# IuvenisSapiens/Qwen3-TTS-Rust

Hardware: AMD Instinct MI355X
Metric: audio-seconds generated per second (aggregate over GPUs) = concurrent real-time streams; RTF and first-chunk latency from the single-utterance leg (higher is better)
Workload: dtype i8

## Files before the change

### qwen3-tts-rust_amd/csrc/codec.hip

```cpp
#include "codec.h"
#include "gguf.h"
#include <cmath>
#include <cstdlib>
#include <map>

namespace q3 {

typedef float f32x16 __attribute__((ext_vector_type(16)));

enum { EPI_NONE = 0, EPI_GELU = 1, EPI_RES_SCALE = 2, EPI_RES = 3, EPI_SNAKE = 4 };

struct GemmArgs {
    const float* A; int lda;
    int cin, dil;
    const float* W;
    const float* bias;
    float* out; int ldo;
    int M, N, K;
    int epi; const float* res; int ldr; const float* scale;
    const float *snake_ea, *snake_ib;
    float* ws;
    int a_segT, a_skip; int o_segT; long long o_skip; int r_segT; long long r_skip;
    int a_split, o_split;
    int xcd_swizzle;
};
#define SEG_NONE 0x3fffffff

__device__ __forceinline__ int seg_of(int row, int segT) { return segT == SEG_NONE ? 0 : row / segT; }
__device__ __forceinline__ size_t out_off(const GemmArgs& g, int row, int col) { return (size_t)row * g.ldo + (size_t)seg_of(row, g.o_segT) * g.o_skip + col; }
typedef _Float16 h4v_ __attribute__((ext_vector_type(4)));
__device__ __forceinline__ float4 load_a4(const GemmArgs& g, size_t row, int ci) {
    if (!g.a_split) return *reinterpret_cast<const float4*>(g.A + row * g.lda + ci);
    const _Float16* base = reinterpret_cast<const _Float16*>(g.A + row * g.lda);
    const h4v_ hi = *reinterpret_cast<const h4v_*>(base + ci), lo = *reinterpret_cast<const h4v_*>(base + g.cin + ci);
    return make_float4((float)hi[0] + (float)lo[0], (float)hi[1] + (float)lo[1], (float)hi[2] + (float)lo[2], (float)hi[3] + (float)lo[3]);
}
__device__ __forceinline__ float4 load_a4_split_raw(const GemmArgs& g, size_t row, int ci) {
    const _Float16* base = reinterpret_cast<const _Float16*>(g.A + row * g.lda);
    const float2 hi = *reinterpret_cast<const float2*>(base + ci), lo = *reinterpret_cast<const float2*>(base + g.cin + ci);
    return make_float4(hi.x, hi.y, lo.x, lo.y);
}
__device__ __forceinline__ void gemm_store(const GemmArgs& g, int row, int col, float v) {
    const size_t o = out_off(g, row, 0);
    if (!g.o_split) { g.out[o + col] = v; return; }
    _Float16* base = reinterpret_cast<_Float16*>(g.out + o);
    const _Float16 hi = (_Float16)v;
    base[col] = hi; base[g.N + col] = (_Float16)(v - (float)hi);
}

__device__ __forceinline__ float snake_sin(float x) {
    const float n = rintf(x * 0.63661977236758134f);
    float r = fmaf(n, -1.57079637050628662f, x);
    r = fmaf(n, 4.37113900018624283e-8f, r);
    const int q = (int)n;
    const float r2 = r * r;
    const float sp = fmaf(fmaf(fmaf(-1.9515295891e-4f, r2, 8.3321608736e-3f), r2, -1.6666654611e-1f), r2 * r, r);
    const float cp = fmaf(fmaf(fmaf(2.443315711809948e-5f, r2, -1.388731625493765e-3f), r2, 4.166664568298827e-2f), r2 * r2, fmaf(-0.5f, r2, 1.0f));
    const float v = (q & 1) ? cp : sp;
    return (q & 2) ? -v : v;
}
__device__ __forceinline__ float gemm_epilogue(const GemmArgs& g, float v, int row, int col) {
    if (g.bias) v += g.bias[col];
    if (g.epi == EPI_GELU) v = 0.5f * v * (1.0f + erff(v * 0.70710678118654752f));
    else if (g.epi == EPI_RES_SCALE) v = g.res[(size_t)row * g.ldr + (size_t)seg_of(row, g.r_segT) * g.r_skip + col] + g.scale[col] * v;
    else if (g.epi == EPI_RES) v = g.res[(size_t)row * g.ldr + (size_t)seg_of(row, g.r_segT) * g.r_skip + col] + v;
    else if (g.epi == EPI_SNAKE) { const float sn = snake_sin(v * g.snake_ea[col]); v = v + g.snake_ib[col] * (sn * sn); }
    return v;
}

typedef _Float16 h4e_ __attribute__((ext_vector_type(4)));
__device__ __forceinline__ void gemm_epilogue_store4(const GemmArgs& g, float4 t, int row, int col) {
    float v[4] = {t.x, t.y, t.z, t.w};
    if (g.bias) { const float4 b = *reinterpret_cast<const float4*>(g.bias + col); v[0] += b.x; v[1] += b.y; v[2] += b.z; v[3] += b.w; }
    if (g.epi == EPI_GELU) {
#pragma unroll
        for (int c = 0; c < 4; c++) v[c] = 0.5f * v[c] * (1.0f + erff(v[c] * 0.70710678118654752f));
    } else if (g.epi == EPI_RES_SCALE || g.epi == EPI_RES) {
        const float4 rs = *reinterpret_cast<const float4*>(g.res + (size_t)row * g.ldr + (size_t)seg_of(row, g.r_segT) * g.r_skip + col);
        if (g.epi == EPI_RES_SCALE) {
            const float4 sc = *reinterpret_cast<const float4*>(g.scale + col);
            v[0] = rs.x + sc.x * v[0]; v[1] = rs.y + sc.y * v[1]; v[2] = rs.z + sc.z * v[2]; v[3] = rs.w + sc.w * v[3];
        } else { v[0] = rs.x + v[0]; v[1] = rs.y + v[1]; v[2] = rs.z + v[2]; v[3] = rs.w + v[3]; }
    } else if (g.epi == EPI_SNAKE) {
        const float4 ea = *reinterpret_cast<const float4*>(g.snake_ea + col), ib = *reinterpret_cast<const float4*>(g.snake_ib + col);
        const float eav[4] = {ea.x, ea.y, ea.z, ea.w}, ibv[4] = {ib.x, ib.y, ib.z, ib.w};
#pragma unroll
        for (int c = 0; c < 4; c++) { const float sn = snake_sin(v[c] * eav[c]); v[c] = v[c] + ibv[c] * (sn * sn); }
    }
    const size_t o = out_off(g, row, 0);
    if (!g.o_split) *reinterpret_cast<float4*>(g.out + o + col) = make_float4(v[0], v[1], v[2], v[3]);
    else {
        _Float16* base = reinterpret_cast<_Float16*>(g.out + o);
        h4e_ hi, lo;
#pragma unroll
        for (int c = 0; c < 4; c++) { hi[c] = (_Float16)v[c]; lo[c] = (_Float16)(v[c] - (float)hi[c]); }
        *reinterpret_cast<h4e_*>(base + col) = hi;
        *reinterpret_cast<h4e_*>(base + g.N + col) = lo;
    }
}
static bool epilogue4_ok(const GemmArgs& g) {
    auto a16 = [](const void* p) { return (reinterpret_cast<uintptr_t>(p) & 15) == 0; };
    return g.N % 4 == 0 && g.ldo % 4 == 0 && g.o_skip % 4 == 0 && a16(g.out) && (!g.bias || a16(g.bias)) &&
           (!(g.epi == EPI_RES || g.epi == EPI_RES_SCALE) || (g.ldr % 4 == 0 && g.r_skip % 4 == 0 && a16(g.res))) &&
           (g.epi != EPI_RES_SCALE || a16(g.scale)) && (g.epi != EPI_SNAKE || (a16(g.snake_ea) && a16(g.snake_ib)));
}

template <int WM>
__global__ void __launch_bounds__(256) k_conv_gemm(GemmArgs g) {
    constexpr int WN = 4 / WM, BM = 32 * WM, BN = 32 * WN, BK = 16;
    constexpr int NA = BM * 4 / 256 > 0 ? BM * 4 / 256 : 1, NB = BN * 4 / 256 > 0 ? BN * 4 / 256 : 1;
    __shared__ float As[BK][BM];
    __shared__ float Bs[BK][BN];
    const int tid = threadIdx.x, lane = tid & 63, wave = tid >> 6;
    const int wm = wave / WN, wn = wave % WN;
    const int m0 = blockIdx.y * BM, n0 = blockIdx.x * BN;
    const int ksplit = gridDim.z, kper = g.K / ksplit, kbeg = blockIdx.z * kper, kend = kbeg + kper;
    f32x16 acc;
#pragma unroll
    for (int i = 0; i < 16; i++) acc[i] = 0.0f;
    float4 ra[NA], rb[NB];
    int arow[NA];
#pragma unroll
    for (int i = 0; i < NA; i++) { const int mm = m0 + (tid + i * 256) % BM; arow[i] = mm + seg_of(mm, g.a_segT) * g.a_skip; }
    auto fetch = [&](int k0) {
        const int j = k0 / g.cin, ci0 = k0 % g.cin;
#pragma unroll
        for (int i = 0; i < NA; i++) {
            const int e = tid + i * 256, r = e % BM, qd = e / BM;
            ra[i] = make_float4(0.f, 0.f, 0.f, 0.f);
            if (e < BM * 4 && m0 + r < g.M) ra[i] = load_a4(g, (size_t)(arow[i] + j * g.dil), ci0 + 4 * qd);
        }
#pragma unroll
        for (int i = 0; i < NB; i++) {
            const int e = tid + i * 256, r = e % BN, qd = e / BN;
            rb[i] = make_float4(0.f, 0.f, 0.f, 0.f);
            if (e < BN * 4 && n0 + r < g.N) rb[i] = *reinterpret_cast<const float4*>(g.W + (size_t)(n0 + r) * g.K + k0 + 4 * qd);
        }
// ... 368 lines not shown
            const int kk = 4 * (lane + 64 * i);
            w4[i] = (kk < kt) ? *reinterpret_cast<const float4*>(g.W + (size_t)nn * g.K + k0 + kk) : make_float4(0.f, 0.f, 0.f, 0.f);
        }
        __syncthreads();
        for (int e = tid; e < MT * (KT / 4); e += 512) {
            const int m = e / (KT / 4), kk = 4 * (e % (KT / 4));
            float4 v = make_float4(0.f, 0.f, 0.f, 0.f);
            if (m < g.M && kk < kt) {
                const int kg = k0 + kk, j = kg / g.cin, ci = kg % g.cin;
                v = load_a4(g, (size_t)(m + seg_of(m, g.a_segT) * g.a_skip + j * g.dil), ci);
            }
            *reinterpret_cast<float4*>(&As[m][kk]) = v;
        }
        __syncthreads();
#pragma unroll
        for (int i = 0; i < 2; i++) {
            const int kk = 4 * (lane + 64 * i);
#pragma unroll
            for (int m = 0; m < MT; m++) {
                const float4 a = *reinterpret_cast<const float4*>(&As[m][kk]);
                acc[m] += w4[i].x * a.x + w4[i].y * a.y + w4[i].z * a.z + w4[i].w * a.w;
            }
        }
    }
    float mine = 0.0f;
#pragma unroll
    for (int m = 0; m < MT; m++) {
        float v = acc[m];
        for (int o = 32; o >= 1; o >>= 1) v += __shfl_xor(v, o);
        if (lane == m) mine = v;
    }
    if (lane < MT && lane < g.M && n < g.N) gemm_store(g, lane, n, gemm_epilogue(g, mine, lane, n));
}
static const bool g_codec_f32 = [] { const char* e = std::getenv("Q3_CODEC_F32"); return e && e[0] == '1'; }();
static void gemm(hipStream_t st, GemmArgs g, float* ws, size_t ws_floats, const _Float16* wh = nullptr, const _Float16* wl = nullptr) {
    if (g.M <= 16) {
        dim3 grid((g.N + 7) / 8);
        if (g.M <= 4) hipLaunchKernelGGL((k_skinny_gemm<4>), grid, dim3(512), 0, st, g);
        else if (g.M <= 8) hipLaunchKernelGGL((k_skinny_gemm<8>), grid, dim3(512), 0, st, g);
        else hipLaunchKernelGGL((k_skinny_gemm<16>), grid, dim3(512), 0, st, g);
        return;
    }
    const bool small = g.M <= 32;
    const int tiles = small ? ((g.N + 127) / 128) * ((g.M + 31) / 32) : ((g.N + 63) / 64) * ((g.M + 63) / 64);
    int ksplit = 1;
    while (tiles * ksplit < 256 && ksplit < 16 && (g.K / (ksplit * 2)) % 16 == 0 && g.K / (ksplit * 2) >= 128 &&
           (size_t)(ksplit * 2) * g.M * g.N <= ws_floats) ksplit *= 2;
    g.ws = ws;
    static const int xcd_on = [] { const char* e = std::getenv("Q3_CODEC_XCD"); return e ? atoi(e) : 1; }();
    g.xcd_swizzle = xcd_on;
    static const int h3_min_wgs = [] { const char* e = std::getenv("Q3_CODEC_H3_MIN_WGS"); return e ? atoi(e) : 128; }();
    static const int h3_max_n = [] { const char* e = std::getenv("Q3_CODEC_H3_MAXN"); return e ? atoi(e) : 1 << 30; }();
    static const int epl_on = [] { const char* e = std::getenv("Q3_CODEC_H3_EPL"); return e ? atoi(e) : 1; }();
    static const int h3_wgs = [] { const char* e = std::getenv("Q3_CODEC_H3_WGS"); return e ? atoi(e) : 0; }();
    static const int h3_min_tiles = [] { const char* e = std::getenv("Q3_CODEC_H3_MIN_TILES"); return e ? atoi(e) : 96; }();
    if (!small && wh && !g_codec_f32 && g.cin % 32 == 0 && h3_min_wgs > 0 && g.N % 96 == 0 && g.N <= h3_max_n) {
        const int tiles3 = (g.N / 96) * ((g.M + 127) / 128);
        const bool vec_ok = epl_on && epilogue4_ok(g) && (reinterpret_cast<uintptr_t>(ws) & 15) == 0;
        int ks = 1;
        if (vec_ok && h3_wgs > 0 && tiles3 >= h3_min_tiles && tiles3 < h3_wgs) {
            static const int cand[] = {2, 3, 4, 6, 7, 8, 12, 14, 16};
            for (int c : cand) {
                if (g.K % c != 0 || (g.K / c) % 32 != 0 || g.K / c < 256 || (size_t)c * g.M * g.N > ws_floats) continue;
                ks = c;
                if (tiles3 * c >= h3_wgs) break;
            }
// ... 253 lines not shown
    }
}
struct ConvW { DevBuf<float> w, b; DevBuf<_Float16> wh, wl; int N = 0, K = 0, cin = 0, taps = 1, dil = 1; };
struct Snake { DevBuf<float> ea, inv_eb; int C = 0; };
struct Ext { DevBuf<float> hist; int H = 0, C = 0, Tmax = 0, id = -1; };

struct CodecDecoder::Impl {
    int n_q, cb_size, cb_dim, hidden, n_layers, n_heads, head_dim, ffn, window, n_up, dec_dim, n_dec;
    int up_ratios[4], dec_rates[8];
    float rope_base, eps;
    int n_streams, max_frames, max_pos = 8192;
    std::vector<DevBuf<float>> codebooks; DevBuf<const float*> d_cb_ptrs;
    ConvW pre_conv;
    struct TfL { DevBuf<float> attn_norm, ffn_norm, ls_attn, ls_ffn; ConvW wqkv, wo, wgu, wdown; };
    std::vector<TfL> tf; DevBuf<float> tf_norm, rope_c, rope_s;
    struct Up { ConvW ct, pw1, pw2; DevBuf<float> dw_w, dw_b, ln_w, ln_b, gamma; };
    std::vector<Up> up;
    ConvW conv_in;
    struct RU { Snake s1, s2; ConvW c1, c2; };
    struct Blk { Snake snake; ConvW ct; RU ru[3]; int cin, cout, rate; };
    std::vector<Blk> blk;
    Snake snake_out; DevBuf<float> conv_out_w; float conv_out_b = 0;
    Ext z_ext, convin_ext, out_ext; std::vector<Ext> dw_ext, ct_ext, k_ext, v_ext; std::vector<std::vector<Ext>> ru_ext;
    std::vector<Ext*> all_ext;
    bool presplit = false;
    std::vector<int> kv_len; std::vector<long long> n_seen;
    int gmax = 1;
    struct Scratch {
        DevBuf<float> h, xn, qkv, att, gu, act, t1, t2, pcm, splitk_ws; DevBuf<int64_t> d_in;
        std::vector<DevBuf<float>> work;
        int64_t* h_in = nullptr; int ring_idx = 0;
    };
    std::vector<Scratch> lanes; Scratch* S = nullptr; int ring = 256;
    size_t in_slot() const { return (size_t)gmax * max_frames * n_q + 3 * (size_t)gmax; }
    double flops_frame = 0;

    static std::vector<float> tensor(const Gguf& g, const std::string& name) {
        const GgufTensor& t = g.need(name);
        Q3_CHECK(t.type == Q3_T_F32, "codec tensor not F32: " + name);
        const float* p = reinterpret_cast<const float*>(t.data);
        return std::vector<float>(p, p + t.nbytes / 4);
    }
    static void up_f(DevBuf<float>& d, const std::vector<float>& v) { d.alloc(v.size()); d.upload(v.data(), v.size()); }
    static void split_w(ConvW& c, const std::vector<float>& r) {
        std::vector<_Float16> h(r.size()), l(r.size());
        for (size_t i = 0; i < r.size(); i++) { h[i] = (_Float16)r[i]; l[i] = (_Float16)(r[i] - (float)h[i]); }
        c.wh.alloc(h.size()); c.wh.upload(h.data(), h.size());
        c.wl.alloc(l.size()); c.wl.upload(l.data(), l.size());
    }
    void make_conv(ConvW& c, const Gguf& g, const std::string& wn, const std::string& bn, int cout, int cin, int k, int dil) {
        auto w = tensor(g, wn);
        Q3_CHECK((int64_t)w.size() == (int64_t)cout * cin * k && cin % 16 == 0, "conv shape " + wn);
        std::vector<float> r((size_t)cout * cin * k);
        for (int co = 0; co < cout; co++) for (int ci = 0; ci < cin; ci++) for (int j = 0; j < k; j++)
            r[((size_t)co * k + j) * cin + ci] = w[((size_t)co * cin + ci) * k + j];
        up_f(c.w, r); split_w(c, r);
        if (!bn.empty()) up_f(c.b, tensor(g, bn));
        c.N = cout; c.K = cin * k; c.cin = cin; c.taps = k; c.dil = dil;
    }
    void make_linear(ConvW& c, const std::vector<float>& w, int N, int K) { up_f(c.w, w); split_w(c, w); c.N = N; c.K = K; c.cin = K; c.taps = 1; c.dil = 1; }
    void make_convt(ConvW& c, const Gguf& g, const std::string& wn, const std::string& bn, int cin, int cout, int k, int s) {
        auto w = tensor(g, wn);
        auto b = tensor(g, bn);
        Q3_CHECK((int64_t)w.size() == (int64_t)cin * cout * k && (k == 2 * s || k == s) && cin % 16 == 0, "convT shape " + wn);
        const int taps = k / s;
        std::vector<float> r((size_t)s * cout * taps * cin), br((size_t)s * cout);
        for (int rr = 0; rr < s; rr++) for (int co = 0; co < cout; co++) {
            br[(size_t)rr * cout + co] = b[co];
            for (int ci = 0; ci < cin; ci++) {
                if (taps == 2) {
                    r[((size_t)(rr * cout + co) * 2 + 0) * cin + ci] = w[((size_t)ci * cout + co) * k + rr + s];
                    r[((size_t)(rr * cout + co) * 2 + 1) * cin + ci] = w[((size_t)ci * cout + co) * k + rr];
                } else r[(size_t)(rr * cout + co) * cin + ci] = w[((size_t)ci * cout + co) * k + rr];
            }
        }
        up_f(c.w, r); split_w(c, r); up_f(c.b, br);
        c.N = s * cout; c.K = taps * cin; c.cin = cin; c.taps = taps; c.dil = 1;
    }
    void make_snake(Snake& s, const Gguf& g, const std::string& an, const std::string& bn, int C) {
        auto a = tensor(g, an), b = tensor(g, bn);
        std::vector<float> ea(C), ib(C);
        for (int i = 0; i < C; i++) { ea[i] = expf(a[i]); ib[i] = 1.0f / (expf(b[i]) + 1e-9f); }
        up_f(s.ea, ea); up_f(s.inv_eb, ib); s.C = C;
    }
    void make_ext(Ext& e, int H, int C, int Tmax) {
        e.H = H; e.C = C; e.Tmax = Tmax; e.id = (int)all_ext.size();
        e.hist.alloc((size_t)n_streams * H * C); e.hist.zero();
        all_ext.push_back(&e);
    }
    struct Loc { float* p; int segT; long long skip_rows; };
    Loc plain(float* p) { return Loc{p, SEG_NONE, 0}; }
    float* work(const Ext& e) { return S->work[e.id].p; }
    Loc ext_base(const Ext& e, int T) { return Loc{work(e), T, e.H}; }
    Loc ext_cur(const Ext& e, int T) { return Loc{work(e) + (size_t)e.H * e.C, T, e.H}; }
    RowMap cur_map(const Ext& e, int T) { return RowMap{T, e.H, e.H}; }
    RowMap base_map(const Ext& e, int T) { return RowMap{T, e.H, 0}; }
    void run_conv(hipStream_t st, const ConvW& c, Loc A, int lda, int M, Loc out, int ldo, int out_C, int epi = EPI_NONE,
                  Loc res = Loc{nullptr, SEG_NONE, 0}, int ldr = 0, const float* scale = nullptr, const Snake* sn = nullptr, bool a_split = false,
                  bool o_split = false) {
        GemmArgs g{};
        g.a_split = a_split ? 1 : 0; g.o_split = o_split ? 1 : 0;
        g.A = A.p; g.lda = lda; g.cin = c.cin; g.dil = c.dil; g.W = c.w.p; g.bias = c.b.n ? c.b.p : nullptr; g.out = out.p; g.ldo = ldo;
        g.M = M; g.N = c.N; g.K = c.K; g.epi = epi; g.res = res.p; g.ldr = ldr; g.scale = scale;
        g.a_segT = A.segT; g.a_skip = (int)A.skip_rows;
        g.o_segT = out.segT; g.o_skip = out.skip_rows * out_C;
        g.r_segT = res.segT; g.r_skip = res.skip_rows * ldr;
        if (sn) { g.snake_ea = sn->ea.p; g.snake_ib = sn->inv_eb.p; }
        gemm(st, g, S->splitk_ws.p, S->splitk_ws.n, c.wh.n ? c.wh.p : nullptr, c.wl.n ? c.wl.p : nullptr);
    }
    HistTable table;
    void plan_hist(const Ext& e, int T) {
        if (e.H == 0) return;
        Q3_CHECK(table.n < 48, "too many streaming convolutions");
        Q3_CHECK(e.C % 4 == 0, "streaming state rows must be a multiple of 4 channels (k_hist_all moves float4s)");
        table.d[table.n++] = HistDesc{work(e), e.hist.p, e.H, e.C, T, 0};
    }
    void move_hist(hipStream_t st, int G, const int64_t* meta, bool save) {
        size_t mx = 0;
        for (int i = 0; i < table.n; i++) mx = std::max(mx, (size_t)table.d[i].H * table.d[i].C);
        hipLaunchKernelGGL(k_hist_all, dim3((unsigned)((mx / 4 + 255) / 256), G, table.n), dim3(256), 0, st, table, meta, save ? 1 : 0);
    }

    void snake(hipStream_t st, const Snake& s, const float* src, float* dst, int rows, RowMap dm, bool split = false) {
        Q3_CHECK(s.C % 4 == 0, "SnakeBeta channel count must be a multiple of 4");
        const size_t n = (size_t)rows * (s.C / 4);
        hipLaunchKernelGGL(k_snake, dim3((unsigned)((n + 255) / 256)), dim3(256), 0, st, src, dst, s.C, s.ea.p, s.inv_eb.p, n, dm, split ? 1 : 0);
    }
    void copy_rows(hipStream_t st, const float* src, float* dst, int rows, int C, RowMap dm) {
        const size_t n = (size_t)rows * C;
        hipLaunchKernelGGL(k_copy_rows, dim3((unsigned)((n + 255) / 256)), dim3(256), 0, st, src, dst, n, C, dm);
    }
};

CodecDecoder::CodecDecoder(const std::string& path, int n_streams, int max_frames, int n_lanes, int max_group) : impl_(new Impl()) {
    Impl& m = *impl_;
    if (const char* e = std::getenv("Q3_CODEC_PRESPLIT")) m.presplit = !(e[0] == '0');
    if (g_codec_f32) m.presplit = false;
    Gguf g(path);
    m.n_streams = n_streams; m.max_frames = max_frames; m.gmax = max_group > 0 ? max_group : 1;
    m.n_q = (int)g.kv_int("codec.n_codebooks", 16); m.cb_size = (int)g.kv_int("codec.codebook_size", 2048);
    m.cb_dim = (int)g.kv_int("codec.codebook_dim", 512); m.hidden = (int)g.kv_int("codec.hidden", 1024);
    m.n_layers = (int)g.kv_int("codec.n_layers", 8); m.n_heads = (int)g.kv_int("codec.n_heads", 16);
    m.head_dim = (int)g.kv_int("codec.head_dim", 64); m.ffn = (int)g.kv_int("codec.ffn", 3072);
    m.window = (int)g.kv_int("codec.window", 72); m.dec_dim = (int)g.kv_int("codec.dec_dim", 1536);
    m.rope_base = (float)g.kv_float("codec.rope_base", 10000.0); m.eps = (float)g.kv_float("codec.eps", 1e-5);
    m.n_up = (int)g.kv_int("codec.n_up", 2); m.n_dec = (int)g.kv_int("codec.n_dec", 4);
    static const int def_rates[8] = {8, 5, 4, 3, 2, 2, 2, 2};
    for (int i = 0; i < m.n_up; i++) m.up_ratios[i] = (int)g.kv_int("codec.up_ratio." + std::to_string(i), 2);
    for (int i = 0; i < m.n_dec; i++) m.dec_rates[i] = (int)g.kv_int("codec.dec_rate." + std::to_string(i), def_rates[i]);
    const int H = m.hidden, A = m.n_heads * m.head_dim;
    Q3_CHECK(A == H && m.head_dim <= 128 && m.window <= 128 && m.cb_dim % 16 == 0 && H % 16 == 0 && m.ffn % 16 == 0, "unsupported codec dims");
    std::vector<const float*> cbp;
    m.codebooks.resize(m.n_q);
    for (int q = 0; q < m.n_q; q++) { Impl::up_f(m.codebooks[q], Impl::tensor(g, "codec.codebook." + std::to_string(q))); cbp.push_back(m.codebooks[q].p); }
    m.d_cb_ptrs.alloc(m.n_q); m.d_cb_ptrs.upload(cbp.data(), m.n_q);
// ... 85 lines not shown
    for (int i = 0; i < m.n_up; i++) { T *= m.up_ratios[i]; m.make_ext(m.dw_ext[i], 6, H, T); }
    const int Tlat = T;
    m.make_ext(m.convin_ext, 6, H, Tlat);
    m.ct_ext.resize(m.n_dec); m.ru_ext.resize(m.n_dec);
    size_t max_act = (size_t)Tlat * 4 * H;
    ch = m.dec_dim;
    static const int dil[3] = {1, 3, 9};
    for (int b = 0; b < m.n_dec; b++) {
        m.make_ext(m.ct_ext[b], 1, ch, T);
        T *= m.dec_rates[b]; ch /= 2;
        m.ru_ext[b].resize(3);
        for (int u = 0; u < 3; u++) m.make_ext(m.ru_ext[b][u], 6 * dil[u], ch, T);
        max_act = std::max(max_act, (size_t)T * ch);
    }
    m.make_ext(m.out_ext, 6, ch, T);
    max_act = std::max(max_act, (size_t)Tlat * m.dec_dim);
    max_act *= GM;
    m.kv_len.assign(n_streams, 0); m.n_seen.assign(n_streams, 0);
    m.lanes.resize(n_lanes > 0 ? n_lanes : 1);
    for (auto& L : m.lanes) {
        const size_t R0 = (size_t)GM * T0;
        L.h.alloc(R0 * H); L.xn.alloc(R0 * H); L.qkv.alloc(R0 * 3 * H); L.att.alloc(R0 * H);
        L.gu.alloc(R0 * 2 * m.ffn); L.act.alloc(R0 * m.ffn);
        L.t1.alloc(max_act); L.t2.alloc(max_act); L.pcm.alloc((size_t)GM * T);
        L.work.resize(m.all_ext.size());
        for (Ext* e : m.all_ext) L.work[e->id].alloc((size_t)GM * (e->H + e->Tmax) * e->C);
        L.d_in.alloc(m.in_slot());
        L.splitk_ws.alloc(std::max<size_t>(max_act * 2, (size_t)1 << 20));
        Q3_HIP(hipHostMalloc((void**)&L.h_in, (size_t)m.ring * m.in_slot() * sizeof(int64_t)));
    }
    m.S = &m.lanes[0];
    Q3_HIP(hipDeviceSynchronize());
}
CodecDecoder::~CodecDecoder() { if (impl_) for (auto& L : impl_->lanes) if (L.h_in) (void)hipHostFree(L.h_in); }
int CodecDecoder::max_group() const { return impl_->gmax; }
int CodecDecoder::n_lanes() const { return (int)impl_->lanes.size(); }
int CodecDecoder::samples_per_frame() const {
    int s = 1;
    for (int i = 0; i < impl_->n_up; i++) s *= impl_->up_ratios[i];
    for (int i = 0; i < impl_->n_dec; i++) s *= impl_->dec_rates[i];
    return s;
}
double CodecDecoder::flops_per_frame() const { return impl_->flops_frame; }

void CodecDecoder::reset(int s) {
    Impl& m = *impl_;
    Q3_CHECK(s >= 0 && s < m.n_streams, "stream out of range");
    std::lock_guard<std::mutex> cap(capture_mutex());
    for (Ext* e : m.all_ext) if (e->H) Q3_HIP(hipMemset(e->hist.p + (size_t)s * e->H * e->C, 0, (size_t)e->H * e->C * 4));
    m.kv_len[s] = 0; m.n_seen[s] = 0;
}

std::vector<CodecStateEntry> CodecDecoder::state_layout() const {
    const Impl& m = *impl_;
    std::vector<CodecStateEntry> out;
    size_t off = 0;
    auto add = [&](const std::string& name, const Ext& e) {
        if (!e.H) return;
        out.push_back(CodecStateEntry{name, (int64_t)off, e.H, e.C});
        off += (size_t)e.H * e.C;
    };
    add("pre_conv_history", m.z_ext);
    for (size_t l = 0; l < m.k_ext.size(); l++) { add("past_key_" + std::to_string(l), m.k_ext[l]); add("past_value_" + std::to_string(l), m.v_ext[l]); }
    for (size_t i = 0; i < m.dw_ext.size(); i++) add("conv_history.upsample." + std::to_string(i), m.dw_ext[i]);
    add("conv_history.conv_in", m.convin_ext);
    for (size_t b = 0; b < m.ct_ext.size(); b++) {
        add("conv_history.block." + std::to_string(b) + ".transposed", m.ct_ext[b]);
// ... 51 lines not shown
    };
    for (Ext* e : m.all_ext) {
        if (!e->H) continue;
        HistDesc d{}; d.hist = e->hist.p; d.H = e->H; d.C = e->C;
        tab.d[tab.n++] = d;
        mx = std::max(mx, (size_t)e->H * e->C);
        if (tab.n == 48) flush();
    }
    flush();
    m.kv_len[s] = 0; m.n_seen[s] = 0;
}

int CodecDecoder::decode(hipStream_t st, int s, const int64_t* codes, int n_frames, bool is_last, float* pcm) {
    const int T = decode_async(st, s, codes, n_frames, is_last, pcm, 0);
    Q3_HIP(hipStreamSynchronize(st));
    return T;
}
int CodecDecoder::decode_async(hipStream_t st, int s, const int64_t* codes, int n_frames, bool is_last, float* pcm, int lane) {
    (void)is_last;
    return decode_group_async(st, 1, &s, codes, n_frames, &pcm, lane);
}

int CodecDecoder::decode_group_async(hipStream_t st, int G, const int* streams, const int64_t* codes, int n_frames, float* const* pcm, int lane) {
    Impl& m = *impl_;
    Q3_CHECK(lane >= 0 && lane < (int)m.lanes.size(), "codec lane out of range");
    Q3_CHECK(G >= 1 && G <= m.gmax, "group size out of range");
    m.S = &m.lanes[lane];
    if (n_frames <= 0) return 0;
    Q3_CHECK(n_frames <= m.max_frames, "too many frames per decode call");
    for (int g = 0; g < G; g++) {
        Q3_CHECK(streams[g] >= 0 && streams[g] < m.n_streams, "stream out of range");
        for (int h = 0; h < g; h++) Q3_CHECK(streams[h] != streams[g], "a stream may appear once per group");
    }
    const int H = m.hidden, T0 = n_frames, R0 = G * T0, W = m.window;
    if (m.S->ring_idx == m.ring) { Q3_HIP(hipStreamSynchronize(st)); m.S->ring_idx = 0; }
    int64_t* hin = m.S->h_in + (size_t)(m.S->ring_idx++) * m.in_slot();
    const size_t ncodes = (size_t)R0 * m.n_q;
    std::copy(codes, codes + ncodes, hin);
    for (int g = 0; g < G; g++) { hin[ncodes + g] = streams[g]; hin[ncodes + G + g] = m.kv_len[streams[g]]; hin[ncodes + 2 * G + g] = m.n_seen[streams[g]]; }
    Q3_HIP(hipMemcpyAsync(m.S->d_in.p, hin, (ncodes + 3 * (size_t)G) * 8, hipMemcpyHostToDevice, st));
    const int64_t* d_codes = m.S->d_in.p;
    const int64_t* meta = m.S->d_in.p + ncodes;
    {
        m.table.n = 0;
        m.plan_hist(m.z_ext, T0);
        for (int l = 0; l < m.n_layers; l++) { m.plan_hist(m.k_ext[l], T0); m.plan_hist(m.v_ext[l], T0); }
        int Tp = T0;
        for (int i = 0; i < m.n_up; i++) { Tp *= m.up_ratios[i]; m.plan_hist(m.dw_ext[i], Tp); }
        m.plan_hist(m.convin_ext, Tp);
        for (int b = 0; b < m.n_dec; b++) {
            m.plan_hist(m.ct_ext[b], Tp);
            Tp *= m.dec_rates[b];
            for (int u = 0; u < 3; u++) m.plan_hist(m.ru_ext[b][u], Tp);
        }
        m.plan_hist(m.out_ext, Tp);
        m.move_hist(st, G, meta, false);
    }
    hipLaunchKernelGGL(k_rvq_sum, dim3((m.cb_dim + 255) / 256, R0), dim3(256), 0, st, d_codes, m.d_cb_ptrs.p, m.n_q, m.cb_size, m.cb_dim,
                       m.work(m.z_ext), m.cb_dim, m.cur_map(m.z_ext, T0));
    m.run_conv(st, m.pre_conv, m.ext_base(m.z_ext, T0), m.cb_dim, R0, m.plain(m.S->h.p), H, H);
    for (int l = 0; l < m.n_layers; l++) {
        auto& L = m.tf[l];
        Ext &ke = m.k_ext[l], &ve = m.v_ext[l];
        hipLaunchKernelGGL(k_rmsnorm_rows, dim3(R0), dim3(256), 0, st, m.S->h.p, H, L.attn_norm.p, H, m.eps, m.S->xn.p, H);
        m.run_conv(st, L.wqkv, m.plain(m.S->xn.p), H, R0, m.plain(m.S->qkv.p), 3 * H, 3 * H);
        hipLaunchKernelGGL(k_codec_rope_append, dim3((H / 2 + 255) / 256, R0), dim3(256), 0, st, m.S->qkv.p, 3 * H, H, m.head_dim, m.rope_c.p, m.rope_s.p,
                           meta, G, T0, m.max_pos, m.work(ke), m.work(ve), m.cur_map(ke, T0));
        hipLaunchKernelGGL(k_codec_attn, dim3(m.n_heads, R0), dim3(64), 0, st, m.S->qkv.p, 3 * H, H, m.head_dim, m.work(ke), m.work(ve), meta, G, T0, W,
                           m.S->att.p, H);
        m.run_conv(st, L.wo, m.plain(m.S->att.p), H, R0, m.plain(m.S->h.p), H, H, EPI_RES_SCALE, m.plain(m.S->h.p), H, L.ls_attn.p);
        hipLaunchKernelGGL(k_rmsnorm_rows, dim3(R0), dim3(256), 0, st, m.S->h.p, H, L.ffn_norm.p, H, m.eps, m.S->xn.p, H);
        m.run_conv(st, L.wgu, m.plain(m.S->xn.p), H, R0, m.plain(m.S->gu.p), 2 * m.ffn, 2 * m.ffn);
        hipLaunchKernelGGL(k_swiglu_rows, dim3((m.ffn + 255) / 256, R0), dim3(256), 0, st, m.S->gu.p, m.ffn, m.S->act.p);
        m.run_conv(st, L.wdown, m.plain(m.S->act.p), m.ffn, R0, m.plain(m.S->h.p), H, H, EPI_RES_SCALE, m.plain(m.S->h.p), H, L.ls_ffn.p);
    }
    for (int g = 0; g < G; g++) {
        const int s = streams[g], tot = m.kv_len[s] + T0;
        m.kv_len[s] = tot < W - 1 ? tot : W - 1;
        m.n_seen[s] += T0;
    }
    hipLaunchKernelGGL(k_rmsnorm_rows, dim3(R0), dim3(256), 0, st, m.S->h.p, H, m.tf_norm.p, H, m.eps, m.S->t1.p, H);
    int T = T0;
    float* x = m.S->t1.p;
    for (int i = 0; i < m.n_up; i++) {
        auto& U = m.up[i];
        const int f = m.up_ratios[i];
        Ext& e = m.dw_ext[i];
        m.run_conv(st, U.ct, m.plain(x), H, G * T, Impl::Loc{m.work(e) + (size_t)e.H * e.C, T, e.H}, f * H, H);
        T *= f;
        hipLaunchKernelGGL(k_dwconv7, dim3((H + 255) / 256, G * T), dim3(256), 0, st, m.work(e), H, U.dw_w.p, U.dw_b.p, m.S->t2.p, m.base_map(e, T));
        hipLaunchKernelGGL(k_layernorm_rows, dim3(G * T), dim3(256), 0, st, m.S->t2.p, H, U.ln_w.p, U.ln_b.p, H, 1e-6f, m.S->t2.p, H);
        float* m1 = m.S->t1.p;
        m.run_conv(st, U.pw1, m.plain(m.S->t2.p), H, G * T, m.plain(m1), 4 * H, 4 * H, EPI_GELU);
        m.run_conv(st, U.pw2, m.plain(m1), 4 * H, G * T, m.plain(m.S->t2.p), H, H, EPI_RES_SCALE, m.ext_cur(e, T), H, U.gamma.p);
        m.copy_rows(st, m.S->t2.p, m.S->t1.p, G * T, H, plain_map());
        x = m.S->t1.p;
    }
    m.copy_rows(st, x, m.work(m.convin_ext), G * T, H, m.cur_map(m.convin_ext, T));
    m.run_conv(st, m.conv_in, m.ext_base(m.convin_ext, T), H, G * T, m.plain(m.S->t1.p), m.dec_dim, m.dec_dim);
    float* d = m.S->t1.p;
    for (int b = 0; b < m.n_dec; b++) {
        auto& B = m.blk[b];
        Ext& ce = m.ct_ext[b];
        m.snake(st, B.snake, d, m.work(ce), G * T, m.cur_map(ce, T), m.presplit);
        float* y = (d == m.S->t1.p) ? m.S->t2.p : m.S->t1.p;
        m.run_conv(st, B.ct, m.ext_base(ce, T), B.cin, G * T, m.plain(y), B.rate * B.cout, B.cout, EPI_NONE, Impl::Loc{nullptr, SEG_NONE, 0}, 0, nullptr, nullptr, m.presplit);
        T *= B.rate;
        for (int u = 0; u < 3; u++) {
            Ext& re = m.ru_ext[b][u];
            auto& R = B.ru[u];
            m.snake(st, R.s1, y, m.work(re), G * T, m.cur_map(re, T), m.presplit);
            float* c1o = d;
            m.run_conv(st, R.c1, m.ext_base(re, T), B.cout, G * T, m.plain(c1o), B.cout, B.cout, EPI_SNAKE, Impl::Loc{nullptr, SEG_NONE, 0}, 0, nullptr, &R.s2, m.presplit, m.presplit);
            m.run_conv(st, R.c2, m.plain(c1o), B.cout, G * T, m.plain(y), B.cout, B.cout, EPI_RES, m.plain(y), B.cout, nullptr, nullptr, m.presplit);
        }
        d = y;
    }
    m.snake(st, m.snake_out, d, m.work(m.out_ext), G * T, m.cur_map(m.out_ext, T));
    if (m.out_ext.C == 96 && T % 128 == 0)
        hipLaunchKernelGGL((k_conv_out_win<96>), dim3(G * T / 128), dim3(256), 0, st, m.work(m.out_ext), m.conv_out_w.p, m.conv_out_b, m.S->pcm.p, G * T, m.base_map(m.out_ext, T));
    else
    hipLaunchKernelGGL(k_conv_out_wave, dim3((G * T + 3) / 4), dim3(256), 0, st, m.work(m.out_ext), m.out_ext.C, m.conv_out_w.p, m.conv_out_b, m.S->pcm.p, G * T,
                       m.base_map(m.out_ext, T));
    m.move_hist(st, G, meta, true);
    Q3_LAUNCH_CHECK();
    for (int g = 0; g < G; g++) Q3_HIP(hipMemcpyAsync(pcm[g], m.S->pcm.p + (size_t)g * T, (size_t)T * 4, hipMemcpyDeviceToHost, st));
    return T;
}

}
```

Measured before the change: 696.9.

## Capture codec decode pass in HIP graphs and fuse snake activations into GEMM epilogues

The codec decode pass is moved into a record_pass function and captured once per (lane, group size, frame count) into a HIP graph, which is then replayed. This cuts per-launch host overhead across the many small kernels. GEMM epilogues gain an optional second store that applies the next SnakeBeta activation and writes straight into the next layer's history buffer, removing the standalone snake kernels and the upsample copy_rows passes. Both paths are on by default behind env flags. The graph caching assumes buffer pointers and history plans stay fixed across calls with the same key.

Result: no change. 692.2 (median of 6 runs) (-0.7%).

```diff
diff --git a/qwen3-tts-rust_amd/csrc/codec.hip b/qwen3-tts-rust_amd/csrc/codec.hip
--- a/qwen3-tts-rust_amd/csrc/codec.hip
+++ b/qwen3-tts-rust_amd/csrc/codec.hip
@@ -3,6 +3,8 @@
 #include <cmath>
 #include <cstdlib>
 #include <map>
+#include <mutex>
+#include <tuple>
 
 namespace q3 {
 
@@ -23,6 +25,8 @@
     int a_segT, a_skip; int o_segT; long long o_skip; int r_segT; long long r_skip;
     int a_split, o_split;
     int xcd_swizzle;
+    float* out2; int o2_C, o2_segT, o2_skip, o2_off, o2_split;
+    const float *s2_ea, *s2_ib;
 };
 #define SEG_NONE 0x3fffffff
 
@@ -39,13 +43,6 @@
     const _Float16* base = reinterpret_cast<const _Float16*>(g.A + row * g.lda);
     const float2 hi = *reinterpret_cast<const float2*>(base + ci), lo = *reinterpret_cast<const float2*>(base + g.cin + ci);
     return make_float4(hi.x, hi.y, lo.x, lo.y);
-}
-__device__ __forceinline__ void gemm_store(const GemmArgs& g, int row, int col, float v) {
-    const size_t o = out_off(g, row, 0);
-    if (!g.o_split) { g.out[o + col] = v; return; }
-    _Float16* base = reinterpret_cast<_Float16*>(g.out + o);
-    const _Float16 hi = (_Float16)v;
-    base[col] = hi; base[g.N + col] = (_Float16)(v - (float)hi);
 }
 
 __device__ __forceinline__ float snake_sin(float x) {
@@ -59,6 +56,35 @@
     const float v = (q & 1) ? cp : sp;
     return (q & 2) ? -v : v;
 }
+__device__ __forceinline__ float* out2_row(const GemmArgs& g, int row, int col, int& c) {
+    int lr = row;
+    c = col;
+    if (g.o2_C != g.N) { const int f = g.N / g.o2_C, q = col / g.o2_C; lr = row * f + q; c = col - q * g.o2_C; }
+    const size_t pr = (size_t)lr + (size_t)(g.o2_segT == SEG_NONE ? 0 : lr / g.o2_segT) * g.o2_skip + g.o2_off;
+    return g.out2 + pr * g.o2_C;
+}
+__device__ __forceinline__ void gemm_store(const GemmArgs& g, int row, int col, float v) {
+    if (g.out) {
+        const size_t o = out_off(g, row, 0);
+        if (!g.o_split) g.out[o + col] = v;
+        else {
+            _Float16* base = reinterpret_cast<_Float16*>(g.out + o);
+            const _Float16 hi = (_Float16)v;
+            base[col] = hi; base[g.N + col] = (_Float16)(v - (float)hi);
+        }
+    }
+    if (g.out2) {
+        int c;
+        float* drow = out2_row(g, row, col, c);
+        const float sn = snake_sin(v * g.s2_ea[c]), y = v + g.s2_ib[c] * (sn * sn);
+        if (!g.o2_split) drow[c] = y;
+        else {
+            _Float16* base = reinterpret_cast<_Float16*>(drow);
+            const _Float16 hi = (_Float16)y;
+            base[c] = hi; base[g.o2_C + c] = (_Float16)(y - (float)hi);
+        }
+    }
+}
 __device__ __forceinline__ float gemm_epilogue(const GemmArgs& g, float v, int row, int col) {
     if (g.bias) v += g.bias[col];
     if (g.epi == EPI_GELU) v = 0.5f * v * (1.0f + erff(v * 0.70710678118654752f));
@@ -87,22 +113,43 @@
 #pragma unroll
         for (int c = 0; c < 4; c++) { const float sn = snake_sin(v[c] * eav[c]); v[c] = v[c] + ibv[c] * (sn * sn); }
     }
-    const size_t o = out_off(g, row, 0);
-    if (!g.o_split) *reinterpret_cast<float4*>(g.out + o + col) = make_float4(v[0], v[1], v[2], v[3]);
-    else {
-        _Float16* base = reinterpret_cast<_Float16*>(g.out + o);
-        h4e_ hi, lo;
-#pragma unroll
-        for (int c = 0; c < 4; c++) { hi[c] = (_Float16)v[c]; lo[c] = (_Float16)(v[c] - (float)hi[c]); }
-        *reinterpret_cast<h4e_*>(base + col) = hi;
-        *reinterpret_cast<h4e_*>(base + g.N + col) = lo;
+    if (g.out) {
+        const size_t o = out_off(g, row, 0);
+        if (!g.o_split) *reinterpret_cast<float4*>(g.out + o + col) = make_float4(v[0], v[1], v[2], v[3]);
+        else {
+            _Float16* base = reinterpret_cast<_Float16*>(g.out + o);
+            h4e_ hi, lo;
+#pragma unroll
+            for (int c = 0; c < 4; c++) { hi[c] = (_Float16)v[c]; lo[c] = (_Float16)(v[c] - (float)hi[c]); }
+            *reinterpret_cast<h4e_*>(base + col) = hi;
+            *reinterpret_cast<h4e_*>(base + g.N + col) = lo;
+        }
+    }
+    if (g.out2) {
+        int c;
+        float* drow = out2_row(g, row, col, c);
+        const float4 ea = *reinterpret_cast<const float4*>(g.s2_ea + c), ib = *reinterpret_cast<const float4*>(g.s2_ib + c);
+        const float eav[4] = {ea.x, ea.y, ea.z, ea.w}, ibv[4] = {ib.x, ib.y, ib.z, ib.w};
+        float y[4];
+#pragma unroll
+        for (int k = 0; k < 4; k++) { const float sn = snake_sin(v[k] * eav[k]); y[k] = v[k] + ibv[k] * (sn * sn); }
+        if (!g.o2_split) *reinterpret_cast<float4*>(drow + c) = make_float4(y[0], y[1], y[2], y[3]);
+        else {
+            _Float16* base = reinterpret_cast<_Float16*>(drow);
+            h4e_ hi, lo;
+#pragma unroll
+            for (int k = 0; k < 4; k++) { hi[k] = (_Float16)y[k]; lo[k] = (_Float16)(y[k] - (float)hi[k]); }
+            *reinterpret_cast<h4e_*>(base + c) = hi;
+            *reinterpret_cast<h4e_*>(base + g.o2_C + c) = lo;
+        }
     }
 }
 static bool epilogue4_ok(const GemmArgs& g) {
     auto a16 = [](const void* p) { return (reinterpret_cast<uintptr_t>(p) & 15) == 0; };
     return g.N % 4 == 0 && g.ldo % 4 == 0 && g.o_skip % 4 == 0 && a16(g.out) && (!g.bias || a16(g.bias)) &&
            (!(g.epi == EPI_RES || g.epi == EPI_RES_SCALE) || (g.ldr % 4 == 0 && g.r_skip % 4 == 0 && a16(g.res))) &&
-           (g.epi != EPI_RES_SCALE || a16(g.scale)) && (g.epi != EPI_SNAKE || (a16(g.snake_ea) && a16(g.snake_ib)));
+           (g.epi != EPI_RES_SCALE || a16(g.scale)) && (g.epi != EPI_SNAKE || (a16(g.snake_ea) && a16(g.snake_ib))) &&
+           (!g.out2 || (g.o2_C % 4 == 0 && a16(g.out2) && a16(g.s2_ea) && a16(g.s2_ib)));
 }
 
 template <int WM>
@@ -537,6 +584,8 @@
     }
     if (lane < MT && lane < g.M && n < g.N) gemm_store(g, lane, n, gemm_epilogue(g, mine, lane, n));
 }
+static const bool g_codec_graph = [] { const char* e = std::getenv("Q3_CODEC_GRAPH"); return !(e && e[0] == '0'); }();
+static const bool g_codec_fuse = [] { const char* e = std::getenv("Q3_CODEC_FUSE"); return !(e && e[0] == '0'); }();
 static const bool g_codec_f32 = [] { const char* e = std::getenv("Q3_CODEC_F32"); return e && e[0] == '1'; }();
 static void gemm(hipStream_t st, GemmArgs g, float* ws, size_t ws_floats, const _Float16* wh = nullptr, const _Float16* wl = nullptr) {
     if (g.M <= 16) {
@@ -856,6 +905,9 @@
         int64_t* h_in = nullptr; int ring_idx = 0;
     };
     std::vector<Scratch> lanes; Scratch* S = nullptr; int ring = 256;
+    struct PassGraph { hipGraph_t graph = nullptr; hipGraphExec_t exec = nullptr; int T = 0; };
+    std::map<std::tuple<int, int, int>, PassGraph> graphs;
+    hipStream_t cap_st = nullptr;
     size_t in_slot() const { return (size_t)gmax * max_frames * n_q + 3 * (size_t)gmax; }
     double flops_frame = 0;
 
@@ -919,9 +971,10 @@
     Loc ext_cur(const Ext& e, int T) { return Loc{work(e) + (size_t)e.H * e.C, T, e.H}; }
     RowMap cur_map(const Ext& e, int T) { return RowMap{T, e.H, e.H}; }
     RowMap base_map(const Ext& e, int T) { return RowMap{T, e.H, 0}; }
+    struct Store2 { const Snake* sn; float* p; RowMap map; bool split; };
     void run_conv(hipStream_t st, const ConvW& c, Loc A, int lda, int M, Loc out, int ldo, int out_C, int epi = EPI_NONE,
                   Loc res = Loc{nullptr, SEG_NONE, 0}, int ldr = 0, const float* scale = nullptr, const Snake* sn = nullptr, bool a_split = false,
-                  bool o_split = false) {
+                  bool o_split = false, const Store2* s2 = nullptr) {
         GemmArgs g{};
         g.a_split = a_split ? 1 : 0; g.o_split = o_split ? 1 : 0;
         g.A = A.p; g.lda = lda; g.cin = c.cin; g.dil = c.dil; g.W = c.w.p; g.bias = c.b.n ? c.b.p : nullptr; g.out = out.p; g.ldo = ldo;
@@ -930,6 +983,11 @@
         g.o_segT = out.segT; g.o_skip = out.skip_rows * out_C;
         g.r_segT = res.segT; g.r_skip = res.skip_rows * ldr;
         if (sn) { g.snake_ea = sn->ea.p; g.snake_ib = sn->inv_eb.p; }
+        if (s2) {
+            Q3_CHECK(s2->sn->C % 4 == 0 && c.N % s2->sn->C == 0, "SnakeBeta second store: channel count must be a multiple of 4 dividing N");
+            g.out2 = s2->p; g.o2_C = s2->sn->C; g.o2_segT = s2->map.segT; g.o2_skip = s2->map.skip; g.o2_off = s2->map.off; g.o2_split = s2->split ? 1 : 0;
+            g.s2_ea = s2->sn->ea.p; g.s2_ib = s2->sn->inv_eb.p;
+        }
         gemm(st, g, S->splitk_ws.p, S->splitk_ws.n, c.wh.n ? c.wh.p : nullptr, c.wl.n ? c.wl.p : nullptr);
     }
     HistTable table;
@@ -945,6 +1003,105 @@
         hipLaunchKernelGGL(k_hist_all, dim3((unsigned)((mx / 4 + 255) / 256), G, table.n), dim3(256), 0, st, table, meta, save ? 1 : 0);
     }
 
+    int record_pass(hipStream_t st, int G, int T0) {
+        const int H = hidden, R0 = G * T0, W = window;
+        const bool fuse = g_codec_fuse;
+        const int64_t* d_codes = S->d_in.p;
+        const int64_t* meta = d_codes + (size_t)R0 * n_q;
+        {
+            table.n = 0;
+            plan_hist(z_ext, T0);
+            for (int l = 0; l < n_layers; l++) { plan_hist(k_ext[l], T0); plan_hist(v_ext[l], T0); }
+            int Tp = T0;
+            for (int i = 0; i < n_up; i++) { Tp *= up_ratios[i]; plan_hist(dw_ext[i], Tp); }
+            plan_hist(convin_ext, Tp);
+            for (int b = 0; b < n_dec; b++) {
+                plan_hist(ct_ext[b], Tp);
+                Tp *= dec_rates[b];
+                for (int u = 0; u < 3; u++) plan_hist(ru_ext[b][u], Tp);
+            }
+            plan_hist(out_ext, Tp);
+            move_hist(st, G, meta, false);
+        }
+        hipLaunchKernelGGL(k_rvq_sum, dim3((cb_dim + 255) / 256, R0), dim3(256), 0, st, d_codes, d_cb_ptrs.p, n_q, cb_size, cb_dim,
+                           work(z_ext), cb_dim, cur_map(z_ext, T0));
+        run_conv(st, pre_conv, ext_base(z_ext, T0), cb_dim, R0, plain(S->h.p), H, H);
+        for (int l = 0; l < n_layers; l++) {
+            auto& L = tf[l];
+            Ext &ke = k_ext[l], &ve = v_ext[l];
+            hipLaunchKernelGGL(k_rmsnorm_rows, dim3(R0), dim3(256), 0, st, S->h.p, H, L.attn_norm.p, H, eps, S->xn.p, H);
+            run_conv(st, L.wqkv, plain(S->xn.p), H, R0, plain(S->qkv.p), 3 * H, 3 * H);
+            hipLaunchKernelGGL(k_codec_rope_append, dim3((H / 2 + 255) / 256, R0), dim3(256), 0, st, S->qkv.p, 3 * H, H, head_dim, rope_c.p, rope_s.p,
+                               meta, G, T0, max_pos, work(ke), work(ve), cur_map(ke, T0));
+            hipLaunchKernelGGL(k_codec_attn, dim3(n_heads, R0), dim3(64), 0, st, S->qkv.p, 3 * H, H, head_dim, work(ke), work(ve), meta, G, T0, W,
+                               S->att.p, H);
+            run_conv(st, L.wo, plain(S->att.p), H, R0, plain(S->h.p), H, H, EPI_RES_SCALE, plain(S->h.p), H, L.ls_attn.p);
+            hipLaunchKernelGGL(k_rmsnorm_rows, dim3(R0), dim3(256), 0, st, S->h.p, H, L.ffn_norm.p, H, eps, S->xn.p, H);
+            run_conv(st, L.wgu, plain(S->xn.p), H, R0, plain(S->gu.p), 2 * ffn, 2 * ffn);
+            hipLaunchKernelGGL(k_swiglu_rows, dim3((ffn + 255) / 256, R0), dim3(256), 0, st, S->gu.p, ffn, S->act.p);
+            run_conv(st, L.wdown, plain(S->act.p), ffn, R0, plain(S->h.p), H, H, EPI_RES_SCALE, plain(S->h.p), H, L.ls_ffn.p);
+        }
+        hipLaunchKernelGGL(k_rmsnorm_rows, dim3(R0), dim3(256), 0, st, S->h.p, H, tf_norm.p, H, eps, S->t1.p, H);
+        int T = T0;
+        float* x = S->t1.p;
+        for (int i = 0; i < n_up; i++) {
+            auto& U = up[i];
+            const int f = up_ratios[i];
+            Ext& e = dw_ext[i];
+            run_conv(st, U.ct, plain(x), H, G * T, Loc{work(e) + (size_t)e.H * e.C, T, e.H}, f * H, H);
+            T *= f;
+            hipLaunchKernelGGL(k_dwconv7, dim3((H + 255) / 256, G * T), dim3(256), 0, st, work(e), H, U.dw_w.p, U.dw_b.p, S->t2.p, base_map(e, T));
+            hipLaunchKernelGGL(k_layernorm_rows, dim3(G * T), dim3(256), 0, st, S->t2.p, H, U.ln_w.p, U.ln_b.p, H, 1e-6f, S->t2.p, H);
+            float* m1 = S->t1.p;
+            run_conv(st, U.pw1, plain(S->t2.p), H, G * T, plain(m1), 4 * H, 4 * H, EPI_GELU);
+            if (fuse) {
+                run_conv(st, U.pw2, plain(m1), 4 * H, G * T, i + 1 == n_up ? ext_cur(convin_ext, T) : plain(S->t2.p), H, H, EPI_RES_SCALE, ext_cur(e, T), H, U.gamma.p);
+                x = S->t2.p;
+            } else {
+                run_conv(st, U.pw2, plain(m1), 4 * H, G * T, plain(S->t2.p), H, H, EPI_RES_SCALE, ext_cur(e, T), H, U.gamma.p);
+                copy_rows(st, S->t2.p, S->t1.p, G * T, H, plain_map());
+                x = S->t1.p;
+            }
+        }
+        if (!fuse || n_up == 0) copy_rows(st, x, work(convin_ext), G * T, H, cur_map(convin_ext, T));
+        auto snake_in = [&](int b, int Tb) {
+            if (b < n_dec) return Store2{&blk[b].snake, work(ct_ext[b]), cur_map(ct_ext[b], Tb), presplit};
+            return Store2{&snake_out, work(out_ext), cur_map(out_ext, Tb), false};
+        };
+        const Store2 s_in0 = snake_in(0, T);
+        run_conv(st, conv_in, ext_base(convin_ext, T), H, G * T, plain(fuse ? nullptr : S->t1.p), dec_dim, dec_dim, EPI_NONE, Loc{nullptr, SEG_NONE, 0}, 0,
+                 nullptr, nullptr, false, false, fuse ? &s_in0 : nullptr);
+        float* d = S->t1.p;
+        for (int b = 0; b < n_dec; b++) {
+            auto& B = blk[b];
+            Ext& ce = ct_ext[b];
+            if (!fuse) snake(st, B.snake, d, work(ce), G * T, cur_map(ce, T), presplit);
+            float* y = (d == S->t1.p) ? S->t2.p : S->t1.p;
+            const Store2 s_ru0{&B.ru[0].s1, work(ru_ext[b][0]), cur_map(ru_ext[b][0], T * B.rate), presplit};
+            run_conv(st, B.ct, ext_base(ce, T), B.cin, G * T, plain(y), B.rate * B.cout, B.cout, EPI_NONE, Loc{nullptr, SEG_NONE, 0}, 0, nullptr, nullptr, presplit,
+                     false, fuse ? &s_ru0 : nullptr);
+            T *= B.rate;
+            for (int u = 0; u < 3; u++) {
+                Ext& re = ru_ext[b][u];
+                auto& R = B.ru[u];
+                if (!fuse) snake(st, R.s1, y, work(re), G * T, cur_map(re, T), presplit);
+                float* c1o = d;
+                run_conv(st, R.c1, ext_base(re, T), B.cout, G * T, plain(c1o), B.cout, B.cout, EPI_SNAKE, Loc{nullptr, SEG_NONE, 0}, 0, nullptr, &R.s2, presplit, presplit);
+                const Store2 s_next = u < 2 ? Store2{&B.ru[u + 1].s1, work(ru_ext[b][u + 1]), cur_map(ru_ext[b][u + 1], T), presplit} : snake_in(b + 1, T);
+                run_conv(st, R.c2, plain(c1o), B.cout, G * T, plain(y), B.cout, B.cout, EPI_RES, plain(y), B.cout, nullptr, nullptr, presplit, false,
+                         fuse ? &s_next : nullptr);
+            }
+            d = y;
+        }
+        if (!fuse) snake(st, snake_out, d, work(out_ext), G * T, cur_map(out_ext, T));
+        if (out_ext.C == 96 && T % 128 == 0)
+            hipLaunchKernelGGL((k_conv_out_win<96>), dim3(G * T / 128), dim3(256), 0, st, work(out_ext), conv_out_w.p, conv_out_b, S->pcm.p, G * T, base_map(out_ext, T));
+        else
+            hipLaunchKernelGGL(k_conv_out_wave, dim3((G * T + 3) / 4), dim3(256), 0, st, work(out_ext), out_ext.C, conv_out_w.p, conv_out_b, S->pcm.p, G * T,
+                               base_map(out_ext, T));
+        move_hist(st, G, meta, true);
+        return T;
+    }
     void snake(hipStream_t st, const Snake& s, const float* src, float* dst, int rows, RowMap dm, bool split = false) {
         Q3_CHECK(s.C % 4 == 0, "SnakeBeta channel count must be a multiple of 4");
         const size_t n = (size_t)rows * (s.C / 4);
@@ -1096,7 +1253,13 @@
     m.S = &m.lanes[0];
     Q3_HIP(hipDeviceSynchronize());
 }
-CodecDecoder::~CodecDecoder() { if (impl_) for (auto& L : impl_->lanes) if (L.h_in) (void)hipHostFree(L.h_in); }
+CodecDecoder::~CodecDecoder() {
+    if (!impl_) return;
+    if (!impl_->graphs.empty()) (void)hipDeviceSynchronize();
+    for (auto& kv : impl_->graphs) { if (kv.second.exec) (void)hipGraphExecDestroy(kv.second.exec); if (kv.second.graph) (void)hipGraphDestroy(kv.second.graph); }
+    if (impl_->cap_st) (void)hipStreamDestroy(impl_->cap_st);
+    for (auto& L : impl_->lanes) if (L.h_in) (void)hipHostFree(L.h_in);
+}
 int CodecDecoder::max_group() const { return impl_->gmax; }
 int CodecDecoder::n_lanes() const { return (int)impl_->lanes.size(); }
 int CodecDecoder::samples_per_frame() const {
@@ -1214,98 +1377,37 @@
         Q3_CHECK(streams[g] >= 0 && streams[g] < m.n_streams, "stream out of range");
         for (int h = 0; h < g; h++) Q3_CHECK(streams[h] != streams[g], "a stream may appear once per group");
     }
-    const int H = m.hidden, T0 = n_frames, R0 = G * T0, W = m.window;
+    const int T0 = n_frames, R0 = G * T0, W = m.window;
     if (m.S->ring_idx == m.ring) { Q3_HIP(hipStreamSynchronize(st)); m.S->ring_idx = 0; }
     int64_t* hin = m.S->h_in + (size_t)(m.S->ring_idx++) * m.in_slot();
     const size_t ncodes = (size_t)R0 * m.n_q;
     std::copy(codes, codes + ncodes, hin);
     for (int g = 0; g < G; g++) { hin[ncodes + g] = streams[g]; hin[ncodes + G + g] = m.kv_len[streams[g]]; hin[ncodes + 2 * G + g] = m.n_seen[streams[g]]; }
     Q3_HIP(hipMemcpyAsync(m.S->d_in.p, hin, (ncodes + 3 * (size_t)G) * 8, hipMemcpyHostToDevice, st));
-    const int64_t* d_codes = m.S->d_in.p;
-    const int64_t* meta = m.S->d_in.p + ncodes;
-    {
-        m.table.n = 0;
-        m.plan_hist(m.z_ext, T0);
-        for (int l = 0; l < m.n_layers; l++) { m.plan_hist(m.k_ext[l], T0); m.plan_hist(m.v_ext[l], T0); }
-        int Tp = T0;
-        for (int i = 0; i < m.n_up; i++) { Tp *= m.up_ratios[i]; m.plan_hist(m.dw_ext[i], Tp); }
-        m.plan_hist(m.convin_ext, Tp);
-        for (int b = 0; b < m.n_dec; b++) {
-            m.plan_hist(m.ct_ext[b], Tp);
-            Tp *= m.dec_rates[b];
-            for (int u = 0; u < 3; u++) m.plan_hist(m.ru_ext[b][u], Tp);
-        }
-        m.plan_hist(m.out_ext, Tp);
-        m.move_hist(st, G, meta, false);
-    }
-    hipLaunchKernelGGL(k_rvq_sum, dim3((m.cb_dim + 255) / 256, R0), dim3(256), 0, st, d_codes, m.d_cb_ptrs.p, m.n_q, m.cb_size, m.cb_dim,
-                       m.work(m.z_ext), m.cb_dim, m.cur_map(m.z_ext, T0));
-    m.run_conv(st, m.pre_conv, m.ext_base(m.z_ext, T0), m.cb_dim, R0, m.plain(m.S->h.p), H, H);
-    for (int l = 0; l < m.n_layers; l++) {
-        auto& L = m.tf[l];
-        Ext &ke = m.k_ext[l], &ve = m.v_ext[l];
-        hipLaunchKernelGGL(k_rmsnorm_rows, dim3(R0), dim3(256), 0, st, m.S->h.p, H, L.attn_norm.p, H, m.eps, m.S->xn.p, H);
-        m.run_conv(st, L.wqkv, m.plain(m.S->xn.p), H, R0, m.plain(m.S->qkv.p), 3 * H, 3 * H);
-        hipLaunchKernelGGL(k_codec_rope_append, dim3((H / 2 + 255) / 256, R0), dim3(256), 0, st, m.S->qkv.p, 3 * H, H, m.head_dim, m.rope_c.p, m.rope_s.p,
-                           meta, G, T0, m.max_pos, m.work(ke), m.work(ve), m.cur_map(ke, T0));
-        hipLaunchKernelGGL(k_codec_attn, dim3(m.n_heads, R0), dim3(64), 0, st, m.S->qkv.p, 3 * H, H, m.head_dim, m.work(ke), m.work(ve), meta, G, T0, W,
-                           m.S->att.p, H);
-        m.run_conv(st, L.wo, m.plain(m.S->att.p), H, R0, m.plain(m.S->h.p), H, H, EPI_RES_SCALE, m.plain(m.S->h.p), H, L.ls_attn.p);
-        hipLaunchKernelGGL(k_rmsnorm_rows, dim3(R0), dim3(256), 0, st, m.S->h.p, H, L.ffn_norm.p, H, m.eps, m.S->xn.p, H);
-        m.run_conv(st, L.wgu, m.plain(m.S->xn.p), H, R0, m.plain(m.S->gu.p), 2 * m.ffn, 2 * m.ffn);
-        hipLaunchKernelGGL(k_swiglu_rows, dim3((m.ffn + 255) / 256, R0), dim3(256), 0, st, m.S->gu.p, m.ffn, m.S->act.p);
-        m.run_conv(st, L.wdown, m.plain(m.S->act.p), m.ffn, R0, m.plain(m.S->h.p), H, H, EPI_RES_SCALE, m.plain(m.S->h.p), H, L.ls_ffn.p);
-    }
+    int T;
+    if (g_codec_graph) {
+        auto it = m.graphs.find(std::make_tuple(lane, G, T0));
+        if (it == m.graphs.end()) {
+            std::lock_guard<std::mutex> cap(capture_mutex());
+            if (!m.cap_st) Q3_HIP(hipStreamCreateWithFlags(&m.cap_st, hipStreamNonBlocking));
+            Impl::PassGraph pg{};
+            (void)hipGetLastError();
+            Q3_HIP(hipStreamBeginCapture(m.cap_st, hipStreamCaptureModeThreadLocal));
+            try { pg.T = m.record_pass(m.cap_st, G, T0); }
+            catch (...) { hipGraph_t dead = nullptr; (void)hipStreamEndCapture(m.cap_st, &dead); if (dead) (void)hipGraphDestroy(dead); throw; }
+            Q3_HIP(hipStreamEndCapture(m.cap_st, &pg.graph));
+            Q3_HIP(hipGraphInstantiate(&pg.exec, pg.graph, nullptr, nullptr, 0));
+            it = m.graphs.emplace(std::make_tuple(lane, G, T0), pg).first;
+        }
+        Q3_HIP(hipGraphLaunch(it->second.exec, st));
+        T = it->second.T;
+    } else T = m.record_pass(st, G, T0);
+    Q3_LAUNCH_CHECK();
     for (int g = 0; g < G; g++) {
         const int s = streams[g], tot = m.kv_len[s] + T0;
         m.kv_len[s] = tot < W - 1 ? tot : W - 1;
         m.n_seen[s] += T0;
     }
-    hipLaunchKernelGGL(k_rmsnorm_rows, dim3(R0), dim3(256), 0, st, m.S->h.p, H, m.tf_norm.p, H, m.eps, m.S->t1.p, H);
-    int T = T0;
-    float* x = m.S->t1.p;
-    for (int i = 0; i < m.n_up; i++) {
-        auto& U = m.up[i];
-        const int f = m.up_ratios[i];
-        Ext& e = m.dw_ext[i];
-        m.run_conv(st, U.ct, m.plain(x), H, G * T, Impl::Loc{m.work(e) + (size_t)e.H * e.C, T, e.H}, f * H, H);
-        T *= f;
-        hipLaunchKernelGGL(k_dwconv7, dim3((H + 255) / 256, G * T), dim3(256), 0, st, m.work(e), H, U.dw_w.p, U.dw_b.p, m.S->t2.p, m.base_map(e, T));
-        hipLaunchKernelGGL(k_layernorm_rows, dim3(G * T), dim3(256), 0, st, m.S->t2.p, H, U.ln_w.p, U.ln_b.p, H, 1e-6f, m.S->t2.p, H);
-        float* m1 = m.S->t1.p;
-        m.run_conv(st, U.pw1, m.plain(m.S->t2.p), H, G * T, m.plain(m1), 4 * H, 4 * H, EPI_GELU);
-        m.run_conv(st, U.pw2, m.plain(m1), 4 * H, G * T, m.plain(m.S->t2.p), H, H, EPI_RES_SCALE, m.ext_cur(e, T), H, U.gamma.p);
-        m.copy_rows(st, m.S->t2.p, m.S->t1.p, G * T, H, plain_map());
-        x = m.S->t1.p;
-    }
-    m.copy_rows(st, x, m.work(m.convin_ext), G * T, H, m.cur_map(m.convin_ext, T));
-    m.run_conv(st, m.conv_in, m.ext_base(m.convin_ext, T), H, G * T, m.plain(m.S->t1.p), m.dec_dim, m.dec_dim);
-    float* d = m.S->t1.p;
-    for (int b = 0; b < m.n_dec; b++) {
-        auto& B = m.blk[b];
-        Ext& ce = m.ct_ext[b];
-        m.snake(st, B.snake, d, m.work(ce), G * T, m.cur_map(ce, T), m.presplit);
-        float* y = (d == m.S->t1.p) ? m.S->t2.p : m.S->t1.p;
-        m.run_conv(st, B.ct, m.ext_base(ce, T), B.cin, G * T, m.plain(y), B.rate * B.cout, B.cout, EPI_NONE, Impl::Loc{nullptr, SEG_NONE, 0}, 0, nullptr, nullptr, m.presplit);
-        T *= B.rate;
-        for (int u = 0; u < 3; u++) {
-            Ext& re = m.ru_ext[b][u];
-            auto& R = B.ru[u];
-            m.snake(st, R.s1, y, m.work(re), G * T, m.cur_map(re, T), m.presplit);
-            float* c1o = d;
-            m.run_conv(st, R.c1, m.ext_base(re, T), B.cout, G * T, m.plain(c1o), B.cout, B.cout, EPI_SNAKE, Impl::Loc{nullptr, SEG_NONE, 0}, 0, nullptr, &R.s2, m.presplit, m.presplit);
-            m.run_conv(st, R.c2, m.plain(c1o), B.cout, G * T, m.plain(y), B.cout, B.cout, EPI_RES, m.plain(y), B.cout, nullptr, nullptr, m.presplit);
-        }
-        d = y;
-    }
-    m.snake(st, m.snake_out, d, m.work(m.out_ext), G * T, m.cur_map(m.out_ext, T));
-    if (m.out_ext.C == 96 && T % 128 == 0)
-        hipLaunchKernelGGL((k_conv_out_win<96>), dim3(G * T / 128), dim3(256), 0, st, m.work(m.out_ext), m.conv_out_w.p, m.conv_out_b, m.S->pcm.p, G * T, m.base_map(m.out_ext, T));
-    else
-    hipLaunchKernelGGL(k_conv_out_wave, dim3((G * T + 3) / 4), dim3(256), 0, st, m.work(m.out_ext), m.out_ext.C, m.conv_out_w.p, m.conv_out_b, m.S->pcm.p, G * T,
-                       m.base_map(m.out_ext, T));
-    m.move_hist(st, G, meta, true);
-    Q3_LAUNCH_CHECK();
     for (int g = 0; g < G; g++) Q3_HIP(hipMemcpyAsync(pcm[g], m.S->pcm.p + (size_t)g * T, (size_t)T * 4, hipMemcpyDeviceToHost, st));
     return T;
 }
```
